# carsonswope/3d-beats

Hardware: AMD Instinct MI355X
Metric: classified Mpix/s on 848x480 depth frames (4 trees, depth 20); % of the bounding roofline level (roofline.bound; HBM: roofline.hbm_frac) (higher is better)
Workload: dtype f32

## Files before the change

### 3d-beats_amd/csrc/rdf_hip.hip

```cpp

#include <hip/hip_runtime.h>
#include <stdint.h>
#include <stdio.h>
#include <stdlib.h>
#include <string.h>
#include <time.h>
#include <unistd.h>

#include <algorithm>
#include <atomic>
#include <map>
#include <tuple>
#include <mutex>
#include <utility>
#include <vector>

#include "../../include/rdf_hip.h"
#include "rdf_device.hpp"

namespace {

constexpr int kGroup = 4;
constexpr int kMaxRowsPerWave = 4;
constexpr int kDefaultLdsBudget = 32700;
constexpr int kDefaultLdsBudget512 = 54600;
constexpr int kDefaultHalo = 32;
constexpr int kMinLdsLevels = 6;
constexpr uint32_t kFlagLeftLeaf = 1u, kFlagRightLeaf = 2u, kFlagExact = 4u;
constexpr int kSchedSlots = 128;
constexpr int kGraphSlots = 384;

constexpr int kSchedStride = 32;
constexpr int kSchedWords = 9 * kSchedStride;
constexpr uint32_t kStealFrom = 2;
constexpr uint32_t kXcdQueuesFrom = 64;
__device__ unsigned int g_sched[kSchedSlots + kGraphSlots][kSchedWords];

struct alignas(16) NodeRec16 {
    uint32_t w[4];
};
struct PackInfo {
    uint32_t exact_nodes;
    float scale;
    uint32_t magic;
    uint32_t deep_choice;
    uint32_t generation;
    uint32_t n_trees, max_depth, n_classes;
    uint32_t pad[24];
};
constexpr uint32_t kPackMagic = 0x52444635u;
struct alignas(64) LastLevelRec {
    NodeRec16 node;
    float pdf_left[4], pdf_right[4];
    uint32_t pad[4];
};
static_assert(sizeof(NodeRec16) == 16 && sizeof(PackInfo) == 128 && sizeof(LastLevelRec) == 64, "record sizes");

__host__ __device__ inline int deep_last_levels(int cpad) { return cpad == 4 ? 2 : 1; }
__host__ __device__ inline size_t deep_lines_before(int n_trees, int R, int Lmin)
{
    return (size_t)n_trees * ((((size_t)1 << R) - ((size_t)1 << Lmin)) / 7u);
}
__host__ __device__ inline size_t deep_total_lines(int n_trees, int max_depth, int cpad)
{
    const int R0 = max_depth - deep_last_levels(cpad);
    return deep_lines_before(n_trees, R0, R0 % 3) + ((size_t)n_trees << R0);
}
__host__ __device__ inline bool deep_possible(int n_trees, int max_depth, int cpad)
{
    return n_trees >= 1 && (cpad == 4 || cpad == 8) && max_depth >= 5 && max_depth <= 24;
}

struct EvalArgs {
    const uint16_t *depth;
    const float *forest;
    const NodeRec16 *packed16;
    const uint16_t *filter;
    uint16_t *labels;
    unsigned long long *stats;
    int stats_wide;
    unsigned int *sched;
    uint32_t n_tiles;
    uint32_t tiles_x;
    uint32_t fold;
    uint32_t tiles_y_n;
    int tw_n, th_n, twp_n;
    int halo_xn;
    uint32_t stage_tw8_n, stage_magic_n;
    uint32_t tiles_y;
    int rows_per_wave;
    uint32_t per_img_l;
    uint32_t per_img_d;
    int W, H, Wl, Hl, r;
    int T, D, C, E;
    int nodes;
    int lds_levels;
    int halo;
    int tw, th, twp;
    uint32_t stage_tw8;
    uint32_t stage_magic;
    uint32_t lds_xchg_off;
    uint32_t lds_nodes_off;
    uint32_t lds_mail_off;
    uint32_t lds_list_off;
    uint32_t lds_slab_off;
    const float *packed_pdf;
    const uint4 *last_level;
    uint32_t last_level_min;
    const uint4 *deep;
    int deep_from;
    int cpad;
    int filter_class;
    int check_empty;
    int keep_if_no_leaf;
    int fill_untouched;
    float s;
    const PackInfo *info;
    uint32_t expect_gen;
    unsigned int *stale_flag;
    uint32_t q_static, q_blocks;
    int q_helper;
};

__device__ __forceinline__ uint32_t child_flags(float l, float r)
{
    return ((l >= -1.0f && l < 0.0f) ? 0u : kFlagLeftLeaf) | ((r >= -1.0f && r < 0.0f) ? 0u : kFlagRightLeaf);
}

__device__ __forceinline__ bool int_offset_ok(float a)
{
    const uint32_t b = __float_as_uint(a);
    return (b << 1) == 0u || (((b >> 23) & 0xFFu) - 40u) <= 107u;
}

__device__ __forceinline__ uint32_t guarded_payload(uint32_t byte)
{
    return (byte & 0xFFu) | ((~byte & 0x80u) << 1);
}

__device__ __forceinline__ int thresh_to_int(float t)
{
    if (t != t) return -65535;
    const float c = fminf(fmaxf(__builtin_ceilf(t), -65535.0f), 65536.0f);
    return (int)c;
}

__device__ __forceinline__ NodeRec16 encode_node(float sux, float suy, float svx, float svy, float thresh,
                                                 float l_next, float r_next)
{
    uint32_t flags = child_flags(l_next, r_next);
    const bool ok = int_offset_ok(sux) && int_offset_ok(suy) && int_offset_ok(svx) && int_offset_ok(svy);
    int nx = 0, ny = 0, mx = 0, my = 0;
    if (ok) {
        nx = (int)__builtin_floorf(sux); ny = (int)__builtin_floorf(suy);
        mx = (int)__builtin_floorf(svx); my = (int)__builtin_floorf(svy);
    } else {
        flags |= kFlagExact;
    }
    const uint32_t t = (uint32_t)thresh_to_int(thresh);
    NodeRec16 r;
    r.w[0] = ((uint32_t)nx << 9) | guarded_payload(t);
    r.w[1] = ((uint32_t)ny << 9) | guarded_payload(t >> 8);
    r.w[2] = ((uint32_t)mx << 9) | guarded_payload(t >> 16);
    r.w[3] = ((uint32_t)my << 9) | guarded_payload(flags);
    return r;
}

__device__ __forceinline__ uint4 select4(bool c, const uint4 a, const uint4 b)
{
    return make_uint4(c ? a.x : b.x, c ? a.y : b.y, c ? a.z : b.z, c ? a.w : b.w);
}

typedef float f4u __attribute__((ext_vector_type(4), aligned(4)));
typedef float f3u __attribute__((ext_vector_type(3), aligned(4)));


struct Node {
    float ax, ay, bx, by;
    uint32_t lo16;
    uint32_t w2;
    uint32_t flags;
};

__device__ __forceinline__ Node decode_node(const uint4 w)
{
    Node n;
    n.ax = (float)(int)w.x;
    n.ay = (float)(int)w.y;
    n.bx = (float)(int)w.z;
    n.by = (float)(int)w.w;
    n.lo16 = __builtin_amdgcn_perm(w.y, w.x, 0x0c0c0400u);
    n.w2 = w.z;
    n.flags = w.w;
    return n;
}

__device__ __forceinline__ void set_threshold(Node &n, int t)
{
    n.lo16 = (uint32_t)t & 0xFFFFu;
    n.w2 = (uint32_t)t >> 16;
}

__device__ __forceinline__ uint32_t walk_step(uint32_t h, int g, uint32_t w2, uint32_t flags)
{
    uint32_t next, t;
    asm("v_cmp_ge_i32_sdwa vcc, sext(%2), sext(%3) src0_sel:WORD_1 src1_sel:BYTE_0\n\t"
        "v_cndmask_b32_e64 %1, 31, 30, vcc\n\t"
        "v_lshlrev_b32_e32 %1, %1, %4\n\t"
        "v_addc_co_u32_e32 %0, vcc, %5, %5, vcc\n\t"
        "v_and_or_b32 %0, %1, %6, %0"
        : "=&v"(next), "=&v"(t)
        : "v"(g), "v"(w2), "v"(flags), "v"(h), "s"(0x80000000u)
        : "vcc");
    return next;
}

template <int NL>
struct EvalArgsN {
    EvalArgs l[NL];
};

template <int BLOCK, bool PACKED, int CMAX, bool STATS, int GROUP, bool COMPACT, int NL = 1, bool TW = false, bool DEEP = false>
__global__ __launch_bounds__(BLOCK, TW ? 8 : DEEP ? 4 : BLOCK == 512 ? 6 : BLOCK == 256 ? 5 : 4) void k_eval_forest(const EvalArgsN<NL> ka)
{
    const uint32_t role = NL > 1 ? blockIdx.x % NL : 0u;
    const uint32_t block_id = NL > 1 ? blockIdx.x / NL : blockIdx.x, n_blocks = NL > 1 ? gridDim.x / NL : gridDim.x;
    const EvalArgs &a = ka.l[role];
    extern __shared__ __align__(16) unsigned char lds_raw[];
    uint16_t *lds_tile = reinterpret_cast<uint16_t *>(lds_raw);
    uint4 *lds_nodes = reinterpret_cast<uint4 *>(lds_raw + a.lds_nodes_off);
    uint32_t *s_tile = reinterpret_cast<uint32_t *>(lds_raw + a.lds_mail_off);
    uint16_t *px_list = reinterpret_cast<uint16_t *>(lds_raw + a.lds_list_off);

    const int tid = threadIdx.x;
    const int lane = tid & 63;
    const int K = a.lds_levels;
    const uint32_t nodes_lds = (1u << K) - 1u;
    constexpr uint32_t kWaves = BLOCK / 64;
    const int rows_per_wave = a.rows_per_wave;
    const uint32_t wave = (uint32_t)tid >> 6;
    const uint32_t tw_T = TW ? (uint32_t)a.T : 1u;
    const uint32_t tw_row = TW ? wave / tw_T : 0u, tw_tree = TW ? wave - tw_row * tw_T : 0u;
    const uint32_t tile_rows = TW ? (kWaves / tw_T) * (uint32_t)rows_per_wave : kWaves * (uint32_t)rows_per_wave;

    const uint32_t lds_pitch = 1u << K;
    constexpr bool kLastLevelTable = PACKED && CMAX == 4 && !TW;
    bool last_from_table = false;
    if (kLastLevelTable && a.last_level) {
        const uint2 t = *reinterpret_cast<const uint2 *>(a.last_level + (((size_t)a.T << (a.D - 1)) << 2));
        last_from_table = t.x == 0u && t.y >= a.last_level_min;
    }
    constexpr int kDeepLast = CMAX == 4 ? 2 : 1;
    bool deep_on = false;
    if (DEEP && a.deep) {
        const uint2 t = *reinterpret_cast<const uint2 *>(a.deep + ((deep_total_lines(a.T, a.D, a.cpad) + 1u) << 3));
        deep_on = (uint32_t)a.deep_from >= t.x && t.y == 0u;
    }
    if (DEEP && deep_on) last_from_table = false;
    const int walk_levels = (DEEP && deep_on) ? a.deep_from : last_from_table ? a.D - 1 : a.D;
    for (uint32_t i = tid; i < (uint32_t)a.T * lds_pitch; i += BLOCK) {
        const uint32_t k = i >> K, h = i & (lds_pitch - 1u);
        if (h == 0u) {
            if (K > 0) lds_nodes[i] = make_uint4(0u, 0u, 0u, 0u);
            continue;
        }
        if (PACKED) {
            lds_nodes[i] = reinterpret_cast<const uint4 *>(a.packed16)[((size_t)k << a.D) + h];
        } else {
            const float *p = a.forest + ((size_t)k * (size_t)a.nodes + (h - 1u)) * (size_t)a.E;
            const NodeRec16 r = encode_node(a.s * p[0], a.s * p[1], a.s * p[2], a.s * p[3], p[4], p[5], p[6]);
            lds_nodes[i] = make_uint4(r.w[0], r.w[1], r.w[2], r.w[3]);
        }
    }
    if (tid == 0) s_tile[2] = s_tile[3] = 0u;
    uint32_t st_px = 0, st_lv = 0, st_lf = 0, st_lds = 0, st_rec = 0, st_leaf = 0, st_far = 0, st_blk = 0;
    auto far_lines = [&](const TileCtx &c, uint32_t cx2, uint32_t cy, bool walking, uint32_t img_byte_off) -> uint32_t {
        const bool in_tile = cx2 < c.tw2 && cy < c.th;
        const uint32_t x2 = cx2 + c.tx0_2, y = cy + c.ty0;
        const bool loads = walking && !in_tile && x2 < c.W2 && y < c.H;
        const uint32_t line = (img_byte_off + __umul24(y, c.W2) + x2) >> 7;
        const uint32_t prev = (uint32_t)__shfl_up((int)line, 1);
        const unsigned long long m = __ballot(loads);
        const bool prev_loads = lane > 0 && ((m >> (lane - 1)) & 1ull) != 0ull;
        return (loads && (!prev_loads || prev != line)) ? 1u : 0u;
    };
    auto lines_of = [&](bool active, uint32_t byte_off) -> uint32_t {
        const uint32_t line = byte_off >> 7;
        const uint32_t prev = (uint32_t)__shfl_up((int)line, 1);
        const unsigned long long m = __ballot(active);
        const bool prev_active = lane > 0 && ((m >> (lane - 1)) & 1ull) != 0ull;
        return (active && (!prev_active || prev != line)) ? 1u : 0u;
    };
    const char *depth_b = reinterpret_cast<const char *>(a.depth);
    uint32_t static_tile = block_id;
    const uint32_t xcc = (uint32_t)__builtin_amdgcn_s_getreg(20 | (31 << 11)) & 7u;
    uint32_t q_empty = 0u;
    const uint32_t q_static = a.q_static ? a.q_static : n_blocks;
    const uint32_t q_blocks = a.q_blocks ? a.q_blocks : n_blocks;
    const uint32_t queued = a.n_tiles > q_static ? a.n_tiles - q_static : 0u;

    for (uint32_t it = 0;; ++it) {
        uint32_t tile;
        if (a.sched) {
            if (it == 0u && !a.q_helper) {
                __syncthreads();
                tile = block_id;
            } else {
                if (queued == 0u) break;
                if (tid == 0) {
                    uint32_t t = a.n_tiles;
                    if (q_static < kXcdQueuesFrom) {
                        const uint32_t got = atomicAdd(a.sched, 1u);
                        if (got < queued) t = q_static + got;
                    } else {
                        const uint32_t reach = (((block_id >> 3) & 15u) == 0u || queued >= 2u * q_static || a.q_helper) ? 7u : kStealFrom;
                        for (uint32_t k = 0; k <= reach; ++k) {
                            const uint32_t q = (xcc + k) & 7u;
                            if ((q_empty >> q) & 1u) continue;
                            const uint32_t lo = (uint32_t)(((unsigned long long)queued * q) >> 3);
                            const uint32_t hi = (uint32_t)(((unsigned long long)queued * (q + 1u)) >> 3);
                            const uint32_t got = lo < hi ? atomicAdd(a.sched + q * kSchedStride, 1u) : hi;
                            if (lo < hi && got < hi - lo) { t = q_static + lo + got; break; }
                            q_empty |= 1u << q;
                        }
                    }
                    s_tile[it & 1u] = t;
                }
                __syncthreads();
                tile = (uint32_t)__builtin_amdgcn_readfirstlane((int)s_tile[it & 1u]);
            }
        } else {
            __syncthreads();
            tile = static_tile;
            static_tile += n_blocks;
        }
        if (tile >= a.n_tiles) break;
        const uint32_t tiles_wide = a.tiles_x * a.tiles_y;
        const uint32_t tiles_per_img = tiles_wide + a.tiles_y_n;
        const uint32_t img = tile / tiles_per_img;
        const uint32_t trem = tile - img * tiles_per_img;
        const bool narrow = trem >= tiles_wide;
        const uint32_t ty = narrow ? trem - tiles_wide : trem / a.tiles_x;
        const uint32_t tx = narrow ? a.tiles_x : trem - ty * a.tiles_x;
        const uint32_t fold = narrow ? a.fold : 1u;
        const uint32_t col_shift = narrow ? (a.fold == 4u ? 4u : 5u) : 6u;
        const uint32_t lane_col = (uint32_t)lane & ((1u << col_shift) - 1u), lane_row = (uint32_t)lane >> col_shift;
        const uint32_t x0 = tx * 64u, y0 = ty * tile_rows * fold;
        const int lx = (int)(x0 + lane_col);
        const uint32_t img_boff = (img * a.per_img_d) << 1;
        const uint32_t img_loff = img * a.per_img_l;
        const int tx0 = (int)x0 * a.r - (narrow ? a.halo_xn : a.halo);
        const int ty0 = (int)y0 * a.r - a.halo;
        const int tw = narrow ? a.tw_n : a.tw, th = narrow ? a.th_n : a.th, twp = narrow ? a.twp_n : a.twp;
        const uint32_t stage_tw8 = narrow ? a.stage_tw8_n : a.stage_tw8, stage_magic = narrow ? a.stage_magic_n : a.stage_magic;

        const TileCtx pc = {depth_b + img_boff,
                            (uint32_t)tw * 2u, (uint32_t)th, (uint32_t)twp * 2u, (uint32_t)a.W * 2u, (uint32_t)a.H,
                            (uint32_t)tx0 * 2u, (uint32_t)ty0};

        if (a.check_empty && tw > 0) {
            bool mine = false;
            for (int sub = 0; sub < rows_per_wave; ++sub) {
                const uint32_t trow = (uint32_t)sub * kWaves + wave;
                if (trow >= tile_rows) break;
                const int ly = (int)(y0 + trow * fold + lane_row);
                if (ly < a.Hl && lx < a.Wl) {
                    const uint32_t i = img_loff + (uint32_t)ly * (uint32_t)a.Wl + (uint32_t)lx;
                    const uint32_t d = *reinterpret_cast<const uint16_t *>(
                        depth_b + (img_boff + ((__umul24((uint32_t)(ly * a.r), (uint32_t)a.W) + (uint32_t)(lx * a.r)) << 1)));
                    bool ok = d != 0u && d != kNoPixel;
                    if (ok && a.filter_class != -1) ok = (int)a.filter[i] == a.filter_class;
                    mine |= ok;
                    if (!ok && a.fill_untouched) a.labels[i] = (uint16_t)kNoPixel;
                }
            }
            if (__any(mine) && lane == 0) s_tile[2u + (it & 1u)] = 1u;
            __syncthreads();
            const uint32_t any_mine = s_tile[2u + (it & 1u)];
            if (tid == 0) s_tile[2u + ((it + 1u) & 1u)] = 0u;
            if (any_mine == 0u) continue;
        }

        if (stage_tw8 > 0u) {
            const uint32_t total = (uint32_t)th * stage_tw8;
            for (uint32_t i = (uint32_t)tid; i < total; i += BLOCK) {
                const uint32_t row = __umulhi(i, stage_magic);
                const uint32_t c = (i - row * stage_tw8) << 3;
                const int gy = ty0 + (int)row, gx = tx0 + (int)c;
                uint4 v = make_uint4(0xFFFFFFFFu, 0xFFFFFFFFu, 0xFFFFFFFFu, 0xFFFFFFFFu);
                if ((uint32_t)gy < (uint32_t)a.H && (uint32_t)gx < (uint32_t)a.W)
                    v = *reinterpret_cast<const uint4 *>(
                        depth_b + (img_boff + ((__umul24((uint32_t)gy, (uint32_t)a.W) + (uint32_t)gx) << 1)));
                *reinterpret_cast<uint4 *>(lds_tile + row * (uint32_t)twp + c) = v;
            }
            __syncthreads();
        } else if (tw > 0) {
            for (int row = (int)wave; row < th; row += (int)kWaves) {
                const int gy = ty0 + row;
                const bool row_in = (uint32_t)gy < (uint32_t)a.H;
                for (int col = lane; col < tw; col += 64) {
                    const int gx = tx0 + col;
                    uint32_t v = kNoPixel;
                    if (row_in && (uint32_t)gx < (uint32_t)a.W)
                        v = *reinterpret_cast<const uint16_t *>(
                            depth_b + (img_boff + ((__umul24((uint32_t)gy, (uint32_t)a.W) + (uint32_t)gx) << 1)));
                    lds_tile[row * twp + col] = (uint16_t)v;
                }
            }
            __syncthreads();
        }

        constexpr bool compact = COMPACT;
        uint32_t *s_cnt = reinterpret_cast<uint32_t *>(px_list + BLOCK * rows_per_wave);
        uint32_t my_rank[kMaxRowsPerWave];
        uint32_t my_valid = 0u;
#pragma unroll
        for (int sub = 0; sub < kMaxRowsPerWave; ++sub) {
            if (sub >= rows_per_wave || !compact) break;
            const uint32_t trow = (uint32_t)sub * kWaves + wave;
            const int ly = (int)(y0 + trow * fold + lane_row);
            bool ok = trow < tile_rows && ly < a.Hl && lx < a.Wl;
            if (ok) {
                const uint32_t i = img_loff + (uint32_t)ly * (uint32_t)a.Wl + (uint32_t)lx;
                if (a.filter_class != -1) ok = (int)a.filter[i] == a.filter_class;
                if (ok) {
                    const uint32_t d = (uint32_t)tprobe_value(tprobe_issue(pc, (uint32_t)(lx * a.r - tx0) * 2u, (uint32_t)(ly * a.r - ty0)));
                    ok = d != 0u && d != kNoPixel;
                }
                if (!ok && a.fill_untouched) a.labels[i] = (uint16_t)kNoPixel;
            }
            const unsigned long long b = __ballot(ok);
            if (lane == 0 && trow < tile_rows) s_cnt[trow] = (uint32_t)__popcll(b);
            my_rank[sub] = (uint32_t)__popcll(b & ((1ull << lane) - 1ull));
            my_valid |= ok ? 1u << sub : 0u;
        }
        uint32_t n_valid = 64u * tile_rows;
        if (compact) {
            __syncthreads();
            n_valid = 0u;
            uint32_t my_base[kMaxRowsPerWave];
            for (uint32_t row = 0; row < tile_rows; ++row) {
#pragma unroll
                for (int sub = 0; sub < kMaxRowsPerWave; ++sub)
                    if (row == (uint32_t)sub * kWaves + wave) my_base[sub] = n_valid;
                n_valid += s_cnt[row];
            }
#pragma unroll
            for (int sub = 0; sub < kMaxRowsPerWave; ++sub) {
                if (sub >= rows_per_wave) break;
                if ((my_valid >> sub) & 1u)
                    px_list[my_base[sub] + my_rank[sub]] = (uint16_t)((((uint32_t)sub * kWaves + wave) << 6) | (uint32_t)lane);
            }
            __syncthreads();
        }

        constexpr uint32_t kDone = 0x80000000u, kIdle = 0xFFFFFFFFu;
        auto add_leaf_pdf = [&](uint32_t hk, int tree, int c0, float (&pdf)[CMAX]) -> bool {
            if (STATS && c0 == 0)
                st_leaf += lines_of((int)hk < 0 && hk != kIdle, PACKED ? (hk & ~kDone) * (uint32_t)(a.cpad * 4) : ((hk & ~kDone) >> 1) * (uint32_t)a.E * 4u);
            if (!((int)hk < 0 && hk != kIdle)) return false;
            const uint32_t leaf = (hk & ~kDone) - 2u;
            if (PACKED) {
                const float4 *pp = reinterpret_cast<const float4 *>(a.packed_pdf) +
                    (((((size_t)tree) << a.D) + (leaf >> 1) + 1u) * 2u + (leaf & 1u)) * (size_t)(a.cpad >> 2) +
                    (size_t)(c0 >> 2);
#pragma unroll
                for (int c = 0; c < CMAX; c += 4) {
                    if (c0 + c < a.cpad) {
                        const float4 v = pp[c >> 2];
                        pdf[c] = pdf[c] + v.x; pdf[c + 1] = pdf[c + 1] + v.y;
                        pdf[c + 2] = pdf[c + 2] + v.z; pdf[c + 3] = pdf[c + 3] + v.w;
                    }
                }
            } else {
                const float *pp = a.forest +
                    ((size_t)tree * (size_t)a.nodes + (leaf >> 1)) * (size_t)a.E +
                    7 + (leaf & 1u) * a.C + c0;
#pragma unroll
                for (int c = 0; c < CMAX; c += 4) {
                    if (c0 + c + 3 < a.C) {
                        const f4u v = *reinterpret_cast<const f4u *>(pp + c);
                        pdf[c] = pdf[c] + v.x; pdf[c + 1] = pdf[c + 1] + v.y;
                        pdf[c + 2] = pdf[c + 2] + v.z; pdf[c + 3] = pdf[c + 3] + v.w;
                    } else {
#pragma unroll
                        for (int e = 0; e < 4; ++e)
                            if (c0 + c + e < a.C) pdf[c + e] = pdf[c + e] + pp[c + e];
                    }
                }
            }
            return true;
        };
        uint32_t tw_h = kIdle, tw_i = 0u;
        bool tw_valid = false;
        for (uint32_t first = TW ? (tw_row < tile_rows ? tw_row * 64u : n_valid) : wave * 64u; first < n_valid; first += BLOCK) {
            const uint32_t slot = first + (uint32_t)lane;
            uint32_t entry = slot;
            bool live = true;
            if (compact) {
                if (slot >= n_valid) {
                    if (!DEEP) continue;
                    live = false;
                }
                entry = px_list[live ? slot : first];
            }
            const int ly = (int)(y0 + (entry >> 6) * fold + ((entry & 63u) >> col_shift));
            const int px = (int)(x0 + (entry & ((1u << col_shift) - 1u)));
            if (!compact && (ly >= a.Hl || px >= a.Wl)) {
                if (!DEEP) continue;
                live = false;
            }
            const uint32_t i = img_loff + (uint32_t)ly * (uint32_t)a.Wl + (uint32_t)px;
            const int x = px * a.r, y = ly * a.r;
            const int xl = x - tx0, yl = y - ty0;
            bool skip = false;
            if (!compact && live && a.filter_class != -1) skip = (int)a.filter[i] != a.filter_class;
            uint32_t d = 0u;
            if (!skip && live) d = (uint32_t)tprobe_value(tprobe_issue(pc, (uint32_t)xl * 2u, (uint32_t)yl));
            if (!compact && live && (skip || d == 0u || d == kNoPixel)) {
                if (a.fill_untouched && (!TW || tw_tree == 0u)) a.labels[i] = (uint16_t)kNoPixel;
                if (!DEEP) continue;
                live = false;
            }
            if (DEEP && !live) d = 1u;
            const float df = (float)d;
            const float r0 = __builtin_amdgcn_rcpf(df);
            const float rcp = __builtin_fmaf(__builtin_fmaf(-df, r0, 1.0f), r0, r0);
            float rcp_s = rcp * (1.0f / kNumScale);
            const float df_s = df * kNumScale;
            uint32_t kx2 = ((uint32_t)xl - kMagicBits) * 2u;
            const uint32_t ky = (uint32_t)yl - kMagicBits;
            pin(kx2);

            float best = 0.0f;
            int best_c = 0;
            bool any_leaf = false;

            for (int c0 = 0; c0 < a.C || c0 == 0; c0 += CMAX) {
                float pdf[CMAX];
#pragma unroll
                for (int c = 0; c < CMAX; ++c) pdf[c] = 0.0f;

                for (int kb = TW ? (int)tw_tree : 0; kb < (TW ? (int)tw_tree + 1 : a.T); kb += GROUP) {
                    uint32_t h[GROUP];
#pragma unroll
                    for (int k = 0; k < GROUP; ++k) h[k] = (live && (kb + k) < a.T) ? 1u : kIdle;

#pragma unroll
                    for (int c = 0; c < CMAX; ++c) pin(pdf[c]);
                    const bool fast_levels = PACKED || K > 0;
                    if (fast_levels) set_round_down(rcp_s);

                    for (int j = 0; j < walk_levels; ++j) {
                        bool any = false;
#pragma unroll
                        for (int k = 0; k < GROUP; ++k) any |= (int)h[k] > 0;
                        if (!__any(any)) break;

                        const bool in_lds = j < K;
                        float df_e = df;
                        if (!PACKED && fast_levels && j == K) set_round_nearest(df_e);
                        Node n[GROUP];
                        uint32_t hn[GROUP];
#pragma unroll
                        for (int k = 0; k < GROUP; ++k) hn[k] = (uint32_t)max((int)h[k], (PACKED || in_lds) ? 0 : 1 << j);
                        if (in_lds) {
#pragma unroll
                            for (int k = 0; k < GROUP; ++k) {
                                const uint32_t tk = (uint32_t)min(kb + k, a.T - 1);
                                n[k] = decode_node(lds_nodes[tk * lds_pitch + hn[k]]);
                                if (STATS && c0 == 0) st_lds += (int)h[k] > 0 ? 1u : 0u;
                            }
                        } else if (PACKED) {
#pragma unroll
                            for (int k = 0; k < GROUP; ++k) {
                                const int tk = min(kb + k, a.T - 1);
                                const char *base = reinterpret_cast<const char *>(a.packed16 + ((size_t)tk << a.D));
                                n[k] = decode_node(*reinterpret_cast<const uint4 *>(base + hn[k] * 16u));
                                if (STATS && c0 == 0) st_rec += lines_of((int)h[k] > 0, hn[k] * 16u);
                            }
                        } else {
#pragma unroll
                            for (int k = 0; k < GROUP; ++k) {
                                const int tk = min(kb + k, a.T - 1);
                                const float *p = a.forest + ((size_t)tk * (size_t)a.nodes + (hn[k] - 1u)) * (size_t)a.E;
                                if (STATS && c0 == 0) st_rec += lines_of((int)h[k] > 0, (hn[k] - 1u) * (uint32_t)a.E * 4u);
                                const f4u uv = *reinterpret_cast<const f4u *>(p);
                                const f3u tf = *reinterpret_cast<const f3u *>(p + 4);
                                n[k].ax = a.s * uv.x; n[k].ay = a.s * uv.y; n[k].bx = a.s * uv.z; n[k].by = a.s * uv.w;
                                set_threshold(n[k], thresh_to_int(tf.x));
                                n[k].flags = child_flags(tf.y, tf.z) | kFlagExact;
                            }
                        }

                        uint32_t ux[GROUP], uy[GROUP], vx[GROUP], vy[GROUP];
                        uint32_t fl = 0u;
#pragma unroll
                        for (int k = 0; k < GROUP; ++k) fl |= n[k].flags;
                        if (__any((fl & kFlagExact) != 0u)) {
                            const bool switch_mode = PACKED || in_lds;
                            if (switch_mode) set_round_nearest(df_e);
                            if (PACKED || in_lds) {
#pragma unroll
                                for (int k = 0; k < GROUP; ++k) {
                                    if (n[k].flags & kFlagExact) {
                                        const int tk = min(kb + k, a.T - 1);
                                        if (a.forest) {
                                            const float s_exact = (PACKED && a.info) ? a.info->scale : a.s;
                                            const float *p = a.forest +
                                                ((size_t)tk * (size_t)a.nodes + (hn[k] - 1u)) * (size_t)a.E;
                                            n[k].ax = s_exact * p[0]; n[k].ay = s_exact * p[1];
                                            n[k].bx = s_exact * p[2]; n[k].by = s_exact * p[3];
                                        } else {
                                            n[k].ax = n[k].ay = n[k].bx = n[k].by = 0.0f;
                                            if (a.stale_flag) __hip_atomic_store(a.stale_flag, 1u, __ATOMIC_RELAXED, __HIP_MEMORY_SCOPE_SYSTEM);
                                        }
                                    }
                                }
                            }
#pragma unroll
                            for (int k = 0; k < GROUP; ++k) {
                                const float den = (n[k].flags & kFlagExact) ? df_e : df_s;
                                ux[k] = (uint32_t)min(max(add_wrap(xl, floor_i32(n[k].ax / den)), -(1 << 30)), (1 << 30) - 1) * 2u;
                                uy[k] = (uint32_t)add_wrap(yl, floor_i32(n[k].ay / den));
                                vx[k] = (uint32_t)min(max(add_wrap(xl, floor_i32(n[k].bx / den)), -(1 << 30)), (1 << 30) - 1) * 2u;
                                vy[k] = (uint32_t)add_wrap(yl, floor_i32(n[k].by / den));
                            }
                            if (switch_mode) {
#pragma unroll
                                for (int k = 0; k < GROUP; ++k) { pin(ux[k]); pin(uy[k]); pin(vx[k]); pin(vy[k]); }
                                set_round_down(ux[0]);
                            }
                        } else {
#pragma unroll
                            for (int k = 0; k < GROUP; ++k) {
                                const f2 nu = {n[k].ax, n[k].ay};
                                const f2 nv = {n[k].bx, n[k].by};
                                const f2 r2 = {rcp_s, rcp_s};
                                const f2 m2 = {kMagic, kMagic};
                                const f2 tu = __builtin_elementwise_fma(nu, r2, m2);
                                const f2 tv = __builtin_elementwise_fma(nv, r2, m2);
                                ux[k] = (__float_as_uint(tu.x) << 1) + kx2;
                                uy[k] = __float_as_uint(tu.y) + ky;
                                vx[k] = (__float_as_uint(tv.x) << 1) + kx2;
                                vy[k] = __float_as_uint(tv.y) + ky;
                            }
                        }

                        TileProbe qu[GROUP], qv[GROUP];
#pragma unroll
                        for (int k = 0; k < GROUP; ++k) {
                            qu[k] = tprobe_issue(pc, ux[k], uy[k]);
                            qv[k] = tprobe_issue(pc, vx[k], vy[k]);
                            if (STATS && c0 == 0) {
                                st_far += far_lines(pc, ux[k], uy[k], (int)h[k] > 0, img_boff);
                                st_far += far_lines(pc, vx[k], vy[k], (int)h[k] > 0, img_boff);
                            }
                        }

#pragma unroll
                        for (int k = 0; k < GROUP; ++k) {
                            const bool walking = (int)h[k] > 0;
                            if (STATS && c0 == 0) st_lv += walking ? 1u : 0u;
                            const int g = tprobe_value(qu[k]) - tprobe_value(qv[k]) - (int)n[k].lo16;
                            const uint32_t next = walk_step(h[k], g, n[k].w2, n[k].flags);
                            h[k] = walking ? next : h[k];
                        }
                    }
                    if constexpr (DEEP) {
                      if (deep_on) {
                        const int R0 = a.D - kDeepLast, Lmin = R0 % 3;
                        const f2 r2 = {rcp_s, rcp_s};
                        const f2 m2 = {kMagic, kMagic};
                        unsigned char *slab = lds_raw + a.lds_slab_off + wave * 8192u;
                        const unsigned char *my_block = slab + ((uint32_t)lane << 7);
                        const uint32_t my_swz = ((uint32_t)lane >> 1) & 7u;
                        const uint32_t src_rec = (((uint32_t)lane & 7u) ^ ((uint32_t)lane >> 4)) << 4;
#pragma unroll
                        for (int k0 = 0; k0 < GROUP; ++k0) {
                            uint32_t hk = h[k0];
                            const int tk = min(kb + k0, a.T - 1);
                            auto fetch_blocks = [&](int R) {
                                const size_t base_at = (deep_lines_before(a.T, R, Lmin) + ((size_t)tk << R) - ((size_t)1 << R)) << 7;
                                const uint32_t off = ((int)hk > 0 ? hk : (1u << R)) << 7;
                                const char *tb = reinterpret_cast<const char *>(a.deep) + base_at;
#pragma unroll
                                for (int k = 0; k < 8; ++k) {
                                    const uint32_t owner_off = (uint32_t)__shfl((int)off, k * 8 + (lane >> 3));
                                    const uint32_t byte = owner_off + (src_rec ^ ((k & 1) ? 64u : 0u));
                                    __builtin_amdgcn_global_load_lds((const __attribute__((address_space(1))) void *)(tb + byte),
                                                                     (__attribute__((address_space(3))) void *)(slab + k * 1024), 16, 0, 0);
                                }
                                if (STATS && c0 == 0) st_blk += (int)hk > 0 ? 1u : 0u;
                                asm volatile("s_waitcnt vmcnt(0)" ::: "memory");
                            };
                            auto slot_of = [&](bool mine, uint32_t rec) -> uint4 {
                                const uint4 v = *reinterpret_cast<const uint4 *>(my_block + ((rec ^ my_swz) << 4));
                                return select4(mine, v, make_uint4(0u, 0u, 0u, 0u));
                            };
                            auto slot = [&](uint32_t rec) -> uint4 { return slot_of((int)hk > 0, rec); };
                            auto level1 = [&](const uint4 rec) {
                                const Node n = decode_node(rec);
                                const f2 nu = {n.ax, n.ay};
                                const f2 nv = {n.bx, n.by};
                                const f2 tu = __builtin_elementwise_fma(nu, r2, m2);
                                const f2 tv = __builtin_elementwise_fma(nv, r2, m2);
                                const TileProbe qu = tprobe_issue(pc, (__float_as_uint(tu.x) << 1) + kx2, __float_as_uint(tu.y) + ky);
                                const TileProbe qv = tprobe_issue(pc, (__float_as_uint(tv.x) << 1) + kx2, __float_as_uint(tv.y) + ky);
                                if (STATS && c0 == 0) {
                                    st_lv += (int)hk > 0 ? 1u : 0u;
                                    st_far += far_lines(pc, (__float_as_uint(tu.x) << 1) + kx2, __float_as_uint(tu.y) + ky, (int)hk > 0, img_boff);
                                    st_far += far_lines(pc, (__float_as_uint(tv.x) << 1) + kx2, __float_as_uint(tv.y) + ky, (int)hk > 0, img_boff);
                                }
                                const int g = tprobe_value(qu) - tprobe_value(qv) - (int)n.lo16;
                                const uint32_t next = walk_step(hk, g, n.w2, n.flags);
                                hk = (int)hk > 0 ? next : hk;
                            };
                            for (int R = a.deep_from; R < R0; R += 3) {
                                if (!__any((int)hk > 0)) break;
                                fetch_blocks(R);
                                level1(slot(0u));
                                const uint32_t sa = hk & 1u;
                                level1(slot(1u + sa));
                                level1(slot(3u + 2u * sa + (hk & 1u)));
                            }
                            bool have = false;
                            uint4 p0 = make_uint4(0u, 0u, 0u, 0u), p1 = make_uint4(0u, 0u, 0u, 0u);
                            if (__any((int)hk > 0)) {
                                fetch_blocks(R0);
                                if (CMAX == 4) {
                                    level1(slot(0u));
                                    const uint32_t sa = hk & 1u;
                                    have = (int)hk > 0;
                                    level1(slot(1u + sa));
                                    p0 = slot_of(have, 3u + 2u * sa + (hk & 1u));
                                } else {
                                    have = (int)hk > 0;
                                    level1(slot(0u));
                                    const uint32_t sb = hk & 1u;
                                    p0 = slot_of(have, 2u + 2u * sb);
                                    p1 = slot_of(have, 3u + 2u * sb);
                                }
                            }
                            const bool early = (int)hk < 0 && hk != kIdle && !have;
                            if (__any(early)) {
                                if (STATS && c0 == 0) st_leaf += lines_of(early, (hk & ~kDone) * (uint32_t)(a.cpad * 4));
                                const uint4 *row = reinterpret_cast<const uint4 *>(a.packed_pdf) +
                                                   (early ? (((size_t)tk << (a.D + 1)) + (hk & ~kDone)) * (size_t)(a.cpad >> 2) : (size_t)0);
                                const uint4 e0 = row[0];
                                p0 = select4(early, e0, p0);
                                if (CMAX == 8) {
                                    const uint4 e1 = row[1];
                                    p1 = select4(early, e1, p1);
                                }
                            }
                            pin(p0.x); pin(p0.y); pin(p0.z); pin(p0.w);
                            if (CMAX == 8) { pin(p1.x); pin(p1.y); pin(p1.z); pin(p1.w); }
                            set_round_nearest(p0.x);
                            pin(p0.y); pin(p0.z); pin(p0.w);
                            if (CMAX == 8) { pin(p1.x); pin(p1.y); pin(p1.z); pin(p1.w); }
                            if (have || early) {
                                if (STATS && c0 == 0) st_lf++;
                                pdf[0] = pdf[0] + __uint_as_float(p0.x); pdf[1] = pdf[1] + __uint_as_float(p0.y);
                                pdf[2] = pdf[2] + __uint_as_float(p0.z); pdf[3] = pdf[3] + __uint_as_float(p0.w);
                                if constexpr (CMAX == 8) {
                                    pdf[4] = pdf[4] + __uint_as_float(p1.x); pdf[5] = pdf[5] + __uint_as_float(p1.y);
                                    pdf[6] = pdf[6] + __uint_as_float(p1.z); pdf[7] = pdf[7] + __uint_as_float(p1.w);
                                }
                                any_leaf = true;
                            }
                            if (k0 + 1 < GROUP) {
#pragma unroll
                                for (int c = 0; c < CMAX; ++c) pin(pdf[c]);
                                set_round_down(pdf[0]);
#pragma unroll
                                for (int c = 1; c < CMAX; ++c) pin(pdf[c]);
                            }
                        }
                        continue;
                      }
                    }
                    if (kLastLevelTable && last_from_table) {
                        bool any_w = false;
#pragma unroll
                        for (int k = 0; k < GROUP; ++k) any_w |= (int)h[k] > 0;
                        if (__any(any_w)) {
                            const uint32_t first = 1u << (a.D - 1);
#pragma unroll
                            for (int k = 0; k < GROUP; ++k) {
                                const bool walking = (int)h[k] > 0;
                                const bool ended = (int)h[k] < 0 && h[k] != kIdle;
                                const uint32_t hn = (uint32_t)max((int)h[k], (int)first);
                                const int tk = min(kb + k, a.T - 1);
                                const uint4 *rec = a.last_level + ((((size_t)tk << (a.D - 1)) + (hn - first)) << 2);
                                const uint4 *leaf = reinterpret_cast<const uint4 *>(a.packed_pdf) + (((size_t)tk << (a.D + 1)) + (h[k] & ~kDone));
                                const uint4 *pp = ended ? leaf : rec + 1;
                                const uint4 *np = walking ? rec : reinterpret_cast<const uint4 *>(a.packed16) + ((size_t)tk << a.D);
                                uint4 w = np[0];
                                float4 pa = *reinterpret_cast<const float4 *>(pp);
                                float4 pb = *reinterpret_cast<const float4 *>(pp + 1);
                                asm volatile("" : "+v"(w.x), "+v"(pa.x), "+v"(pb.x));
                                const Node n = decode_node(w);
                                const f2 nu = {n.ax, n.ay};
                                const f2 nv = {n.bx, n.by};
                                const f2 r2 = {rcp_s, rcp_s};
                                const f2 m2 = {kMagic, kMagic};
                                const f2 tu = __builtin_elementwise_fma(nu, r2, m2);
                                const f2 tv = __builtin_elementwise_fma(nv, r2, m2);
                                const TileProbe qu = tprobe_issue(pc, (__float_as_uint(tu.x) << 1) + kx2, __float_as_uint(tu.y) + ky);
                                const TileProbe qv = tprobe_issue(pc, (__float_as_uint(tv.x) << 1) + kx2, __float_as_uint(tv.y) + ky);
                                if (STATS && c0 == 0) {
                                    st_lv += walking ? 1u : 0u;
                                    st_rec += lines_of(walking, (hn - first) * 64u);
                                    st_leaf += lines_of(ended, (h[k] & ~kDone) * 16u);
                                    st_far += far_lines(pc, (__float_as_uint(tu.x) << 1) + kx2, __float_as_uint(tu.y) + ky, walking, img_boff);
                                    st_far += far_lines(pc, (__float_as_uint(tv.x) << 1) + kx2, __float_as_uint(tv.y) + ky, walking, img_boff);
                                }
                                const int g = tprobe_value(qu) - tprobe_value(qv) - (int)n.lo16;
                                const uint32_t next = walk_step(h[k], g, n.w2, n.flags);
                                const bool right = walking && (next & 1u) != 0u;
                                float4 sel = make_float4(right ? pb.x : pa.x, right ? pb.y : pa.y, right ? pb.z : pa.z, right ? pb.w : pa.w);
                                pin(sel.x); pin(sel.y); pin(sel.z); pin(sel.w);
                                set_round_nearest(sel.x);
                                pin(sel.y); pin(sel.z); pin(sel.w);
                                if (walking || ended) {
                                    pdf[0] = pdf[0] + sel.x; pdf[1] = pdf[1] + sel.y;
                                    pdf[2] = pdf[2] + sel.z; pdf[3] = pdf[3] + sel.w;
                                    any_leaf = true;
                                    if (STATS && c0 == 0) st_lf++;
                                }
                                if (k + 1 < GROUP) {
#pragma unroll
                                    for (int c = 0; c < CMAX; ++c) pin(pdf[c]);
                                    set_round_down(pdf[0]);
#pragma unroll
                                    for (int c = 1; c < CMAX; ++c) pin(pdf[c]);
                                }
                            }
                            continue;
                        }
                    }
                    if (fast_levels) {
#pragma unroll
                        for (int k = 0; k < GROUP; ++k) pin(h[k]);
                        set_round_nearest(h[0]);
#pragma unroll
                        for (int k = 0; k < GROUP; ++k) pin(h[k]);
                    }

                    if (TW) { tw_h = h[0]; break; }
                    if (PACKED && CMAX == 4) {
                        float4 row[GROUP];
#pragma unroll
                        for (int k = 0; k < GROUP; ++k) {
                            const bool ended = (int)h[k] < 0 && h[k] != kIdle;
                            const int tk = min(kb + k, a.T - 1);
                            const size_t at = ((((size_t)tk << (a.D + 1)) + (h[k] & ~kDone)) * (size_t)(a.cpad >> 2)) + (size_t)(c0 >> 2);
                            row[k] = reinterpret_cast<const float4 *>(a.packed_pdf)[ended ? at : 0];
                            if (STATS && c0 == 0) st_leaf += lines_of(ended, (uint32_t)at * 16u);
                        }
#pragma unroll
                        for (int k = 0; k < GROUP; ++k) {
                            if ((int)h[k] < 0 && h[k] != kIdle) {
                                pdf[0] = pdf[0] + row[k].x; pdf[1] = pdf[1] + row[k].y;
                                pdf[2] = pdf[2] + row[k].z; pdf[3] = pdf[3] + row[k].w;
                                any_leaf = true;
                                if (STATS && c0 == 0) st_lf++;
                            }
                        }
                    } else {
#pragma unroll
                        for (int k = 0; k < GROUP; ++k) {
                            if (add_leaf_pdf(h[k], kb + k, c0, pdf)) {
                                any_leaf = true;
                                if (STATS && c0 == 0) st_lf++;
                            }
                        }
                    }
                }
                if (TW) break;

#pragma unroll
                for (int c = 0; c < CMAX; ++c) {
                    if (c0 + c < a.C && pdf[c] > best) {
                        best = pdf[c];
                        best_c = c0 + c;
                    }
                }
            }

            if (TW) { tw_valid = true; tw_i = i; continue; }
            if (DEEP && !live) continue;
            if (STATS) st_px++;
            if (a.keep_if_no_leaf && !any_leaf) {
                if (a.fill_untouched) a.labels[i] = (uint16_t)kNoPixel;
                continue;
            }
            a.labels[i] = (uint16_t)best_c;
        }
        if (TW) {
            uint32_t *xch = reinterpret_cast<uint32_t *>(lds_raw + a.lds_xchg_off);
            if (tw_row < tile_rows) xch[(tw_row * tw_T + tw_tree) * 64u + (uint32_t)lane] = tw_valid ? tw_h : kIdle;
            __syncthreads();
            if (tw_row < tile_rows && tw_tree == 0u && tw_valid) {
                float best = 0.0f;
                int best_c = 0;
                bool any_leaf = false;
                for (int c0 = 0; c0 < a.C || c0 == 0; c0 += CMAX) {
                    float pdf[CMAX];
#pragma unroll
                    for (int c = 0; c < CMAX; ++c) pdf[c] = 0.0f;
                    for (uint32_t t = 0; t < tw_T; ++t)
                        any_leaf |= add_leaf_pdf(xch[(tw_row * tw_T + t) * 64u + (uint32_t)lane], (int)t, c0, pdf);
#pragma unroll
                    for (int c = 0; c < CMAX; ++c) {
                        if (c0 + c < a.C && pdf[c] > best) {
                            best = pdf[c];
                            best_c = c0 + c;
                        }
                    }
                }
                if (a.keep_if_no_leaf && !any_leaf) {
                    if (a.fill_untouched) a.labels[tw_i] = (uint16_t)kNoPixel;
                } else {
                    a.labels[tw_i] = (uint16_t)best_c;
                }
            }
        }
    }

    if (PACKED && a.info && a.stale_flag && block_id == n_blocks - 1u && tid == 0 && !a.q_helper) {
        if (a.info->generation != a.expect_gen)
            __hip_atomic_store(a.stale_flag, 1u, __ATOMIC_RELAXED, __HIP_MEMORY_SCOPE_SYSTEM);
    }

    if (a.sched && queued != 0u && tid == 0) {
        const unsigned int done = atomicAdd(a.sched + 8 * kSchedStride, 1u);
        if (done == q_blocks - 1u) {
            for (int q = 0; q < 9; ++q) atomicExch(a.sched + q * kSchedStride, 0u);
        }
    }

    if (STATS) {
        uint32_t c[8] = {st_px, st_lv, st_lf, st_lds, st_rec, st_leaf, st_far, st_blk};
#pragma unroll
        for (int i = 0; i < 8; ++i) {
            unsigned long long v = c[i];
            for (int o = 32; o > 0; o >>= 1) v += __shfl_down(v, o);
            if (lane == 0 && (i < 3 || a.stats_wide)) atomicAdd(a.stats + i, v);
        }
    }
}

__global__ __launch_bounds__(256) void k_pack(const float *forest, NodeRec16 *packed16, PackInfo *info,
                                              float *packed_pdf, LastLevelRec *last_level, unsigned int *last_level_unusable,
                                              uint4 *deep, int n_trees, int C, int cpad,
                                              size_t total_slots, int D, int E, float s, int force_exact, uint32_t generation)
{
    const size_t slot = (size_t)blockIdx.x * 256 + threadIdx.x;
    if (slot >= total_slots) return;
    const size_t tree = slot >> D, h = slot & (((size_t)1 << D) - 1);
    if (h == 0) {
        NodeRec16 z16 = {{0u, 0u, 0u, 0u}};
        packed16[slot] = z16;
        for (int c = 0; c < 2 * cpad; ++c) packed_pdf[slot * 2 * (size_t)cpad + c] = 0.f;
        if (tree == 0) {
            info->scale = s; info->magic = kPackMagic; info->generation = generation;
            info->n_trees = (uint32_t)n_trees; info->max_depth = (uint32_t)D; info->n_classes = (uint32_t)C;
        }
        if (deep && tree == 0) {
            uint4 *z = deep + (deep_total_lines(n_trees, D, cpad) << 3);
            for (int i = 0; i < 8; ++i) z[i] = make_uint4(0u, 0u, 0u, 0u);
        }
        return;
    }
    const size_t i = tree * ((((size_t)1) << D) - 1) + (h - 1);
    const float *p = forest + i * (size_t)E;
    struct { uint32_t flags; } n;
    NodeRec16 h16 = encode_node(s * p[0], s * p[1], s * p[2], s * p[3], p[4], p[5], p[6]);
    if (force_exact) h16.w[3] |= kFlagExact;
    n.flags = h16.w[3] & 0xFFu;
    packed16[slot] = h16;
    if (n.flags & kFlagExact) atomicAdd(&info->exact_nodes, 1u);
    float *q = packed_pdf + slot * 2 * (size_t)cpad;
    for (int c = 0; c < cpad; ++c) {
        q[c] = c < C ? p[7 + c] : 0.f;
        q[cpad + c] = c < C ? p[7 + C + c] : 0.f;
    }
    if (deep) {
        const int R0 = D - deep_last_levels(cpad), Lmin = R0 % 3;
        const int j = 63 - __clzll((unsigned long long)h);
        if (j >= Lmin) {
            const int R = j >= R0 ? R0 : R0 - 3 * ((R0 - j + 2) / 3);
            const int t = j - R;
            const size_t line = deep_lines_before(n_trees, R, Lmin) + (tree << R) + ((h >> t) - ((size_t)1 << R));
            uint4 *blk = deep + (line << 3);
            const uint4 rec = make_uint4(h16.w[0], h16.w[1], h16.w[2], h16.w[3]);
            const float4 *pq = reinterpret_cast<const float4 *>(q);
            const uint4 z = make_uint4(0u, 0u, 0u, 0u);
            if (R == R0 && cpad == 8) {
                blk[0] = rec; blk[1] = z; blk[6] = z; blk[7] = z;
                for (int i = 0; i < 4; ++i) reinterpret_cast<float4 *>(blk)[2 + i] = pq[i];
            } else {
                blk[((1u << t) - 1u) + (uint32_t)(h & ((1u << t) - 1u))] = rec;
                if (t == 0) blk[7] = z;
                if (R == R0 && t == 1) {
                    const uint32_t c = (uint32_t)(h & 1u);
                    reinterpret_cast<float4 *>(blk)[3 + 2 * c] = pq[0];
                    reinterpret_cast<float4 *>(blk)[4 + 2 * c] = pq[1];
                }
            }
            unsigned int *tr = reinterpret_cast<unsigned int *>(deep + ((deep_total_lines(n_trees, D, cpad) + 1u) << 3));
            if (n.flags & kFlagExact) atomicMax(tr, (unsigned)j + 1u);
            if (j == D - 1 && (n.flags & 7u) != (kFlagLeftLeaf | kFlagRightLeaf)) atomicAdd(tr + 1, 1u);
        }
    }
    const size_t first = (size_t)1 << (D - 1);
    if (last_level && h >= first) {
        LastLevelRec r;
        r.node = h16;
        for (int c = 0; c < 4; ++c) {
            r.pdf_left[c] = q[c];
            r.pdf_right[c] = q[4 + c];
            r.pad[c] = 0u;
        }
        last_level[(tree << (D - 1)) + (h - first)] = r;
        const bool unusable = (n.flags & 7u) != (kFlagLeftLeaf | kFlagRightLeaf);
        const float *pp = forest + (tree * ((((size_t)1) << D) - 1) + ((h >> 1) - 1)) * (size_t)E;
        const float to_me = pp[5 + (h & 1)];
        const bool in_use = to_me >= -1.0f && to_me < 0.0f;
        const unsigned long long bu = __ballot(unusable), bi = __ballot(in_use);
        const unsigned long long mine = __ballot(true);
        if ((unsigned)__lane_id() == (unsigned)__ffsll((long long)mine) - 1u) {
            if (bu) atomicAdd(last_level_unusable, (unsigned)__popcll(bu));
            if (bi) atomicAdd(last_level_unusable + 1, (unsigned)__popcll(bi));
        }
    }
}

constexpr int kMaxSpecLayers = 4;
struct SpecFilters {
    int n;
    int fl[kMaxSpecLayers], fc[kMaxSpecLayers];
};

__global__ __launch_bounds__(256) void k_composite(const uint16_t *const *imgs, int n_images, uint32_t n_px,
                                                   const int2 *cond, int n_cond, uint16_t *out, int32_t *bad,
                                                   int fill_untouched, uint32_t flip_w, const uint32_t *colors,
                                                   int num_colors, uint32_t *rgba, const SpecFilters spec)
{
    const uint32_t p = blockIdx.x * 256u + threadIdx.x;
    if (p >= n_px) return;
    uint32_t lab[kMaxSpecLayers];
    if (spec.n > 0) {
#pragma unroll
        for (int i = 0; i < kMaxSpecLayers; ++i) {
            lab[i] = kNoPixel;
            if (i < spec.n) {
                uint32_t l = imgs[i][p];
                if (spec.fl[i] >= 0) {
                    uint32_t f = kNoPixel;
#pragma unroll
                    for (int j = 0; j < kMaxSpecLayers; ++j)
                        if (j < i && j == spec.fl[i]) f = lab[j];
                    if ((int)f != spec.fc[i] && l != kNoPixel) {
                        l = kNoPixel;
                        const_cast<uint16_t *>(imgs[i])[p] = (uint16_t)kNoPixel;
                    }
                }
                lab[i] = l;
            }
        }
    }
    uint32_t q = p;
    if (flip_w) {
        const uint32_t y = p / flip_w, x = p - y * flip_w;
        q = y * flip_w + (flip_w - 1u - x);
    }
    long long off = 0;
    bool invalid = true;
    for (int i = 0; i < n_images; ++i) {
        uint32_t l;
        if (spec.n > 0) {
            l = kNoPixel;
#pragma unroll
            for (int j = 0; j < kMaxSpecLayers; ++j)
                if (j == i) l = lab[j];
        } else {
            l = imgs[i][p];
        }
        if (l == 0u || l == kNoPixel) { invalid = false; break; }
        const long long e = off + (long long)l - 1;
        if (e < 0 || e >= n_cond) break;
        const int2 tv = cond[e];
        if (tv.x == 0) {
            const uint32_t v = (uint32_t)(uint16_t)tv.y;
            out[q] = (uint16_t)v;
            if (rgba && v != 0u && v != kNoPixel && v <= (uint32_t)num_colors) rgba[q] = colors[v - 1u];
            return;
        }
        off = tv.y;
    }
    if (invalid && bad) atomicAdd(bad, 1);
    if (fill_untouched) out[q] = (uint16_t)kNoPixel;
}

__global__ __launch_bounds__(256) void k_fill_u16(uint16_t *dst, size_t n, uint16_t v)
{
    const size_t gid = (size_t)blockIdx.x * 256 + threadIdx.x;
    const size_t stride = (size_t)gridDim.x * 256;
    const uintptr_t addr = reinterpret_cast<uintptr_t>(dst);
    size_t head = ((16 - (addr & 15)) & 15) / 2;
    if (head > n) head = n;
    const size_t nvec = (n - head) / 8;
    const uint32_t w = (uint32_t)v | ((uint32_t)v << 16);
    uint4 *vp = reinterpret_cast<uint4 *>(dst + head);
    for (size_t i = gid; i < nvec; i += stride) vp[i] = make_uint4(w, w, w, w);
    const size_t tail0 = head + nvec * 8;
    for (size_t i = gid; i < head; i += stride) dst[i] = v;
    for (size_t i = tail0 + gid; i < n; i += stride) dst[i] = v;
}

__global__ __launch_bounds__(256) void k_debug_fat(unsigned long long spin_ticks, unsigned long long *t_start)
{
    __shared__ unsigned int pad[19744 / 4];
    asm volatile("v_mov_b32 v250, 0" ::: "v250");
    pad[threadIdx.x] = threadIdx.x;
    __syncthreads();
    const unsigned long long t0 = wall_clock64();
    if (threadIdx.x == 0 && t_start) t_start[blockIdx.x] = t0;
    while (wall_clock64() - t0 < spin_ticks) __builtin_amdgcn_s_sleep(8);
    if (pad[(threadIdx.x + 1) & 255] == 0xFFFFFFFFu && t_start) t_start[0] = 0;
}

__global__ void k_debug_floor(const float *in, int32_t *out, size_t n)
{
    const size_t i = (size_t)blockIdx.x * blockDim.x + threadIdx.x;
    if (i < n) out[i] = floor_i32(in[i]);
}

__global__ void k_debug_div(const float *num, const float *den, float *out, size_t n)
{
    const size_t i = (size_t)blockIdx.x * blockDim.x + threadIdx.x;
    if (i < n) out[i] = num[i] / den[i];
}

struct Knob {
    const int unset;
    const char *const env;
    std::atomic<int> value;
    std::once_flag env_once;
    int env_set = 0, env_val = 0;
    Knob(int unset_, const char *env_) : unset(unset_), env(env_), value(unset_) {}
    int get(int dflt, bool *by_setter = nullptr)
    {
        const int v = value;
        if (by_setter) *by_setter = v > unset;
        if (v > unset) return v;
        if (!env) return dflt;
        std::call_once(env_once, [this]() {
            const char *s = getenv(env);
            if (s && *s) { env_set = 1; env_val = atoi(s); }
        });
        return env_set ? env_val : dflt;
    }
};
Knob g_compaction{-1, nullptr};
Knob g_group{0, nullptr};
Knob g_force_exact{0, nullptr};
Knob g_sched_mode{-1, nullptr};
Knob g_lds_budget{0, nullptr}, g_env_lds_budget{-1, "RDF_LDS_BUDGET"}, g_env_coop_lds_budget{-1, "RDF_COOP_LDS_BUDGET"};
Knob g_env_check_empty_small{-1, "RDF_CHECK_EMPTY_SMALL"};
Knob g_env_last_level_min_pct{-1, "RDF_LAST_LEVEL_MIN_PCT"};
Knob g_block_threads{0, "RDF_BLOCK"};
Knob g_rows_per_wave{0, "RDF_ROWS_PER_WAVE"};
Knob g_halo{-1, "RDF_HALO"};
Knob g_lds_levels{-1, "RDF_LDS_LEVELS"};
Knob g_tree_waves{-1, "RDF_TREE_WAVES"};
Knob g_stage_vec{-1, "RDF_STAGE_VEC"};
Knob g_layers_one_launch{-1, "RDF_LAYERS_ONE_LAUNCH"};
Knob g_fold{-1, "RDF_FOLD"};
Knob g_deep_from{-1, "RDF_DEEP_FROM"};
Knob g_last_level_table{-1, "RDF_LAST_LEVEL_TABLE"};

std::atomic<unsigned long long> g_host_ns_plan{0}, g_host_ns_launch{0}, g_host_calls{0}, g_host_ns_layered{0}, g_host_layered_calls{0};
inline unsigned long long now_ns()
{
    struct timespec ts;
    clock_gettime(CLOCK_MONOTONIC, &ts);
    return (unsigned long long)ts.tv_sec * 1000000000ull + (unsigned long long)ts.tv_nsec;
}

int coop_lds_budget(int block)
{
    const int knob = g_lds_budget.get(0);
    const int v = knob > 0 ? knob : g_env_coop_lds_budget.get(0);
    if (v > 0) return v;
    return block == 512 ? 81920 - 65536 - 1024 : 40960 - 32768 - 1024;
}

int lds_budget(int block)
{
    const int knob = g_lds_budget.get(0);
    int b = knob > 0 ? knob : g_env_lds_budget.get(block == 512 ? kDefaultLdsBudget512 : kDefaultLdsBudget);
    if (b > 160 * 1024) b = 160 * 1024;
    if (b < 0) b = 0;
    return b;
}

struct DeviceInfo {
    int cus = 0, dev = 0;
    bool ok = false;
};

std::atomic<int> g_device_cus[64];

int device_info(DeviceInfo *out)
{
    int dev = 0;
    hipError_t e = hipGetDevice(&dev);
    if (e != hipSuccess) return (int)e;
    int cus = (dev >= 0 && dev < 64) ? g_device_cus[dev].load(std::memory_order_relaxed) : 0;
    if (cus == 0) {
        e = hipDeviceGetAttribute(&cus, hipDeviceAttributeMultiprocessorCount, dev);
        if (e != hipSuccess) return (int)e;
        cus = cus > 0 ? cus : 256;
        if (dev >= 0 && dev < 64) g_device_cus[dev].store(cus, std::memory_order_relaxed);
    }
    out->cus = cus;
    out->dev = dev;
    out->ok = true;
// ... 1295 lines not shown
```

Before: 13640.

## Add scout wave that prefetches and skips empty tiles while block finishes

Restructures the tile scheduling loop for non-TW kernels. The first wave to finish a tile becomes a scout: it pulls the next tile from the queue, tests it for valid pixels with a single wave, and fills the labels of empty tiles itself, so the whole block only synchronises on tiles with work. The emptiness check is vectorised with four row loads in flight and clamped indices. The aim is to hide scheduling and empty-tile overhead behind other waves' work, at the cost of more control complexity, extra LDS slots, and one wave doing serial queue pulls.

```diff
diff --git a/3d-beats_amd/csrc/rdf_hip.hip b/3d-beats_amd/csrc/rdf_hip.hip
--- a/3d-beats_amd/csrc/rdf_hip.hip
+++ b/3d-beats_amd/csrc/rdf_hip.hip
@@ -272,7 +272,7 @@
             lds_nodes[i] = make_uint4(r.w[0], r.w[1], r.w[2], r.w[3]);
         }
     }
-    if (tid == 0) s_tile[2] = s_tile[3] = 0u;
+    if (tid == 0) s_tile[2] = s_tile[3] = s_tile[4] = s_tile[5] = s_tile[6] = 0u;
     uint32_t st_px = 0, st_lv = 0, st_lf = 0, st_lds = 0, st_rec = 0, st_leaf = 0, st_far = 0, st_blk = 0;
     auto far_lines = [&](const TileCtx &c, uint32_t cx2, uint32_t cy, bool walking, uint32_t img_byte_off) -> uint32_t {
         const bool in_tile = cx2 < c.tw2 && cy < c.th;
@@ -292,60 +292,145 @@
         return (active && (!prev_active || prev != line)) ? 1u : 0u;
     };
     const char *depth_b = reinterpret_cast<const char *>(a.depth);
-    uint32_t static_tile = block_id;
     const uint32_t xcc = (uint32_t)__builtin_amdgcn_s_getreg(20 | (31 << 11)) & 7u;
-    uint32_t q_empty = 0u;
     const uint32_t q_static = a.q_static ? a.q_static : n_blocks;
     const uint32_t q_blocks = a.q_blocks ? a.q_blocks : n_blocks;
     const uint32_t queued = a.n_tiles > q_static ? a.n_tiles - q_static : 0u;
 
-    for (uint32_t it = 0;; ++it) {
-        uint32_t tile;
-        if (a.sched) {
-            if (it == 0u && !a.q_helper) {
-                __syncthreads();
-                tile = block_id;
-            } else {
-                if (queued == 0u) break;
-                if (tid == 0) {
-                    uint32_t t = a.n_tiles;
-                    if (q_static < kXcdQueuesFrom) {
-                        const uint32_t got = atomicAdd(a.sched, 1u);
-                        if (got < queued) t = q_static + got;
-                    } else {
-                        const uint32_t reach = (((block_id >> 3) & 15u) == 0u || queued >= 2u * q_static || a.q_helper) ? 7u : kStealFrom;
-                        for (uint32_t k = 0; k <= reach; ++k) {
-                            const uint32_t q = (xcc + k) & 7u;
-                            if ((q_empty >> q) & 1u) continue;
-                            const uint32_t lo = (uint32_t)(((unsigned long long)queued * q) >> 3);
-                            const uint32_t hi = (uint32_t)(((unsigned long long)queued * (q + 1u)) >> 3);
-                            const uint32_t got = lo < hi ? atomicAdd(a.sched + q * kSchedStride, 1u) : hi;
-                            if (lo < hi && got < hi - lo) { t = q_static + lo + got; break; }
-                            q_empty |= 1u << q;
-                        }
-                    }
-                    s_tile[it & 1u] = t;
-                }
-                __syncthreads();
-                tile = (uint32_t)__builtin_amdgcn_readfirstlane((int)s_tile[it & 1u]);
-            }
-        } else {
-            __syncthreads();
-            tile = static_tile;
-            static_tile += n_blocks;
-        }
-        if (tile >= a.n_tiles) break;
+    struct TilePlace { uint32_t img, x0, y0, fold, col_shift; bool narrow; };
+    auto place_tile = [&](uint32_t tile) -> TilePlace {
         const uint32_t tiles_wide = a.tiles_x * a.tiles_y;
         const uint32_t tiles_per_img = tiles_wide + a.tiles_y_n;
-        const uint32_t img = tile / tiles_per_img;
-        const uint32_t trem = tile - img * tiles_per_img;
-        const bool narrow = trem >= tiles_wide;
-        const uint32_t ty = narrow ? trem - tiles_wide : trem / a.tiles_x;
-        const uint32_t tx = narrow ? a.tiles_x : trem - ty * a.tiles_x;
-        const uint32_t fold = narrow ? a.fold : 1u;
-        const uint32_t col_shift = narrow ? (a.fold == 4u ? 4u : 5u) : 6u;
+        TilePlace p;
+        p.img = tile / tiles_per_img;
+        const uint32_t trem = tile - p.img * tiles_per_img;
+        p.narrow = trem >= tiles_wide;
+        const uint32_t ty = p.narrow ? trem - tiles_wide : trem / a.tiles_x;
+        const uint32_t tx = p.narrow ? a.tiles_x : trem - ty * a.tiles_x;
+        p.fold = p.narrow ? a.fold : 1u;
+        p.col_shift = p.narrow ? (a.fold == 4u ? 4u : 5u) : 6u;
+        p.x0 = tx * 64u, p.y0 = ty * tile_rows * p.fold;
+        return p;
+    };
+    auto rows_have_pixels = [&](const TilePlace &p, uint32_t first, uint32_t step, bool store_fails) -> bool {
+        const uint32_t lane_col = (uint32_t)lane & ((1u << p.col_shift) - 1u), lane_row = (uint32_t)lane >> p.col_shift;
+        const uint32_t lx = p.x0 + lane_col;
+        const int y_last = min(a.Hl, (int)(p.y0 + tile_rows * p.fold)) - 1;
+        const uint32_t img_boff = (p.img * a.per_img_d) << 1, img_loff = p.img * a.per_img_l;
+        const uint32_t dy = step * p.fold;
+        uint32_t ly = p.y0 + first * p.fold + lane_row;
+        uint32_t seen = 0u;
+        if ((int)lx < a.Wl) {
+#pragma clang loop unroll(disable)
+            for (uint32_t trow = first; trow < tile_rows; trow += 4u * step, ly += 4u * dy) {
+                uint32_t i[4], d[4];
+#pragma unroll
+                for (uint32_t k = 0; k < 4u; ++k) {
+                    const uint32_t y = (uint32_t)min((int)(ly + k * dy), y_last);
+                    i[k] = img_loff + y * (uint32_t)a.Wl + lx;
+                    d[k] = *reinterpret_cast<const uint16_t *>(
+                        depth_b + (img_boff + ((__umul24(y * (uint32_t)a.r, (uint32_t)a.W) + lx * (uint32_t)a.r) << 1)));
+                }
+                if (a.filter_class != -1) {
+                    uint32_t f[4];
+#pragma unroll
+                    for (uint32_t k = 0; k < 4u; ++k) f[k] = a.filter[i[k]];
+#pragma unroll
+                    for (uint32_t k = 0; k < 4u; ++k) d[k] = (int)f[k] == a.filter_class ? d[k] : 0u;
+                }
+#pragma unroll
+                for (uint32_t k = 0; k < 4u; ++k) {
+                    d[k] = (d[k] + 1u) & 0xFFFFu;
+                    seen = max(seen, d[k]);
+                    if (store_fails && d[k] <= 1u) a.labels[i[k]] = (uint16_t)kNoPixel;
+                }
+            }
+        }
+        return seen > 1u;
+    };
+    auto fill_tile = [&](const TilePlace &p) {
+        const uint32_t lane_col = (uint32_t)lane & ((1u << p.col_shift) - 1u), lane_row = (uint32_t)lane >> p.col_shift;
+        const int lx = (int)(p.x0 + lane_col);
+#pragma clang loop vectorize(disable) unroll(disable)
+        for (uint32_t trow = 0; trow < tile_rows; ++trow) {
+            const int ly = (int)(p.y0 + trow * p.fold + lane_row);
+            if (ly < a.Hl && lx < a.Wl) a.labels[p.img * a.per_img_l + (uint32_t)ly * (uint32_t)a.Wl + (uint32_t)lx] = (uint16_t)kNoPixel;
+        }
+    };
+    auto pull_tile = [&](uint32_t after, uint32_t &q_empty) -> uint32_t {
+        if (!a.sched) return after + n_blocks < a.n_tiles ? after + n_blocks : a.n_tiles;
+        uint32_t t = a.n_tiles;
+        if (q_static < kXcdQueuesFrom) {
+            const uint32_t got = atomicAdd(a.sched, 1u);
+            if (got < queued) t = q_static + got;
+        } else {
+            const uint32_t reach = (((block_id >> 3) & 15u) == 0u || queued >= 2u * q_static || a.q_helper) ? 7u : kStealFrom;
+            for (uint32_t k = 0; k <= reach; ++k) {
+                const uint32_t q = (xcc + k) & 7u;
+                if ((q_empty >> q) & 1u) continue;
+                const uint32_t lo = (uint32_t)(((unsigned long long)queued * q) >> 3);
+                const uint32_t hi = (uint32_t)(((unsigned long long)queued * (q + 1u)) >> 3);
+                const uint32_t got = lo < hi ? atomicAdd(a.sched + q * kSchedStride, 1u) : hi;
+                if (lo < hi && got < hi - lo) { t = q_static + lo + got; break; }
+                q_empty |= 1u << q;
+            }
+        }
+        return t;
+    };
+    const bool more_tiles = a.sched ? queued != 0u : block_id + n_blocks < a.n_tiles;
+    bool scout = !TW && a.sched && a.q_helper && wave == 0u;
+    uint32_t q_empty = 0u;
+    uint32_t tile = block_id;
+
+    for (uint32_t it = 0;; ++it) {
+        const bool own_tile = it == 0u && !(a.sched && a.q_helper);
+        if (!own_tile && !more_tiles) break;
+        if (TW) {
+            if (!own_tile && tid == 0) s_tile[it & 1u] = pull_tile(tile, q_empty);
+        } else {
+            if (own_tile && a.check_empty) __syncthreads();
+            if (scout || (own_tile && a.check_empty)) {
+                uint32_t t = tile;
+                q_empty = s_tile[6];
+                for (;;) {
+                    if (!own_tile) {
+                        if (lane == 0) t = pull_tile(t, q_empty);
+                        t = (uint32_t)__builtin_amdgcn_readfirstlane((int)t);
+                    }
+                    if (t >= a.n_tiles || !a.check_empty) break;
+                    const TilePlace p = place_tile(t);
+                    const bool any = (p.narrow ? a.tw_n : a.tw) <= 0 ||
+                                     __any(rows_have_pixels(p, own_tile ? wave : 0u, own_tile ? kWaves : 1u, own_tile && a.fill_untouched));
+                    if (own_tile) {
+                        if (any && lane == 0) s_tile[2] = 1u;
+                        break;
+                    }
+                    if (any) break;
+                    if (a.fill_untouched) fill_tile(p);
+                }
+                if (!own_tile && lane == 0) {
+                    s_tile[it & 1u] = t;
+                    s_tile[6] = q_empty;
+                }
+            }
+            scout = false;
+        }
+        __syncthreads();
+        if (!own_tile) {
+            tile = (uint32_t)__builtin_amdgcn_readfirstlane((int)s_tile[it & 1u]);
+            if (!TW && tid == 0) s_tile[4u + ((it + 1u) & 1u)] = 0u;
+        }
+        if (tile >= a.n_tiles) break;
+        if (!TW && own_tile && a.check_empty && s_tile[2] == 0u) {
+            scout = wave == 0u;
+            continue;
+        }
+        const TilePlace tp = place_tile(tile);
+        const uint32_t img = tp.img;
+        const bool narrow = tp.narrow;
+        const uint32_t fold = tp.fold, col_shift = tp.col_shift;
         const uint32_t lane_col = (uint32_t)lane & ((1u << col_shift) - 1u), lane_row = (uint32_t)lane >> col_shift;
-        const uint32_t x0 = tx * 64u, y0 = ty * tile_rows * fold;
+        const uint32_t x0 = tp.x0, y0 = tp.y0;
         const int lx = (int)(x0 + lane_col);
         const uint32_t img_boff = (img * a.per_img_d) << 1;
         const uint32_t img_loff = img * a.per_img_l;
@@ -358,7 +443,7 @@
                             (uint32_t)tw * 2u, (uint32_t)th, (uint32_t)twp * 2u, (uint32_t)a.W * 2u, (uint32_t)a.H,
                             (uint32_t)tx0 * 2u, (uint32_t)ty0};
 
-        if (a.check_empty && tw > 0) {
+        if (TW && a.check_empty && tw > 0) {
             bool mine = false;
             for (int sub = 0; sub < rows_per_wave; ++sub) {
                 const uint32_t trow = (uint32_t)sub * kWaves + wave;
@@ -927,6 +1012,11 @@
                 }
             }
         }
+        if (!TW && more_tiles) {
+            uint32_t before = 0u;
+            if (lane == 0) before = atomicAdd(&s_tile[4u + (it & 1u)], 1u);
+            scout = __builtin_amdgcn_readfirstlane((int)before) == 0;
+        }
     }
 
     if (PACKED && a.info && a.stale_flag && block_id == n_blocks - 1u && tid == 0 && !a.q_helper) {
```

Result: faster. 13900, median of 6 (+1.9%).
